# tuplex/tuplex

Measured on AMD Instinct MI355X. Metric: rows/s, higher is better.
Workload: dtype u8; 1 GPU; zillow-Z1 csv->map/withColumn/filter->tocsv (BASELINE.json configs[1]); mb_per_gpu=1024, sink=csv-device-resident

## Files before the change

__graft_entry__.py:

```python
import os
import subprocess
import sys

HERE = os.path.dirname(os.path.abspath(__file__))
sys.path.insert(0, HERE)


def build() -> None:
    from tuplex_amd.csrc import build as nb
    nb.build()
    import tuplex_amd
    subprocess.check_call([sys.executable, os.path.abspath(__file__),
                           "precompile"], cwd=HERE,
                          stdin=subprocess.DEVNULL)
    mk = os.path.join(HERE, "oracle", "Makefile")
    if os.path.exists(mk):
        subprocess.check_call(["make", "-C", os.path.join(HERE, "oracle"), "-s"])


def _precompile() -> None:
    from tests import (chunk_order_pipelines, fused_pipelines, pipelines,
                       regex_pipelines, vocab_pipelines)
    pipelines._COLLECTOR = jobs = []
    try:
        pipelines.precompile_all(verbose=False)
        pipelines.precompile_extra(verbose=False)
        regex_pipelines.precompile(verbose=False)
        chunk_order_pipelines.precompile(verbose=False)
        vocab_pipelines.precompile(verbose=False)
        fused_pipelines.precompile(verbose=False)
    finally:
        pipelines._COLLECTOR = None
    n = pipelines.compile_collected(jobs)
    print("precompiled %d stage kernels into tuplex_amd/.kernel_cache" % n)


def smoke() -> None:
    import tuplex_amd
    from oracle import pyoracle
    from tests.pipelines import PIPELINES, apply_ops

    name, data, columns, ops = PIPELINES[0]
    ctx = tuplex_amd.Context()
    ds = apply_ops(ctx.parallelize(data, columns=columns), ops)
    got = ds.collect()
    assert ds._last_outcome.mode == "gpu", (
        "smoke must run the GPU path, got %r (%s)"
        % (ds._last_outcome.mode, ds._last_outcome.fallback_reason))
    ref = pyoracle.run_pipeline(data, ops, columns=columns)
    assert got == ref["output"], (got, ref["output"])
    assert ds.exception_counts == ref["exception_counts"]
    print("smoke ok:", got)


if __name__ == "__main__":
    if len(sys.argv) > 1 and sys.argv[1] == "smoke":
        smoke()
    elif len(sys.argv) > 1 and sys.argv[1] == "precompile":
        _precompile()
    else:
        build()
```

tuplex_amd/codegen.py:

```python
import os
from typing import List, Optional, Tuple

from . import ttypes as T


class CodegenError(Exception):
    """Stage outside the GPU vocabulary -> caller falls back to interpreter mode
    (the reference's fallback for non-compilable stages)."""


_RT_HEADER_CACHE = None


def runtime_header() -> str:
    global _RT_HEADER_CACHE
    if _RT_HEADER_CACHE is None:
        path = os.path.join(os.path.dirname(os.path.abspath(__file__)),
                            "csrc", "tpx_rt.hip.h")
        _RT_HEADER_CACHE = open(path).read()
    return _RT_HEADER_CACHE


_RE_HEADER_CACHE = None


def regex_header() -> str:
    global _RE_HEADER_CACHE
    if _RE_HEADER_CACHE is None:
        path = os.path.join(os.path.dirname(os.path.abspath(__file__)),
                            "csrc", "tpx_re.hip.h")
        _RE_HEADER_CACHE = open(path).read()
    return _RE_HEADER_CACHE


_FMT_HEADER_CACHE = None


def fmt_header() -> str:
    global _FMT_HEADER_CACHE
    if _FMT_HEADER_CACHE is None:
        path = os.path.join(os.path.dirname(os.path.abspath(__file__)),
                            "csrc", "tpx_fmt.hip.h")
        _FMT_HEADER_CACHE = open(path).read()
    return _FMT_HEADER_CACHE


def _ctype(t):
    base = T.deopt(t)
    if base in (T.I64,):
        return "long long"
    if base == T.F64:
        return "double"
    if base == T.BOOL:
        return "bool"
    if base == T.STR:
        return "tstr"
    raise CodegenError("unsupported column type %r" % (t,))


def _esc(s: str) -> str:
    out = []
    for ch in s:
        o = ord(ch)
        if ch == "\\":
            out.append("\\\\")
        elif ch == '"':
            out.append('\\"')
        elif 32 <= o < 127:
            out.append(ch)
        else:
            for b in ch.encode("utf-8"):
                out.append("\\x%02x" % b)
    return "".join(out)


class _Emitter:
    def __init__(self):
        self.lines: List[str] = []
        self.indent = 1
        self.ctr = 0
        self.scopes = [{}]
        self.key_scopes = [{}]

    def w(self, line):
        self.lines.append("    " * self.indent + line)

    def fresh(self, pfx="t"):
        self.ctr += 1
        return "%s%d" % (pfx, self.ctr)

    def push(self):
        self.scopes.append({})
        self.key_scopes.append({})

    def pop(self):
        self.scopes.pop()
        self.key_scopes.pop()

    def lookup(self, node):
        for s in reversed(self.scopes):
            if id(node) in s:
                return s[id(node)]
        return None

    def memo(self, node, val):
        self.scopes[-1][id(node)] = val
        return val

    def lookup_key(self, key):
        for s in reversed(self.key_scopes):
            if key in s:
                return s[key]
        return None

    def memo_key(self, key, val):
        self.key_scopes[-1][key] = val
        return val


class StageCodegen:

    def __init__(self, sp, source="mem", sink="mem", csv_info=None,
                 fusion_groups=None):
        self.sp = sp
        self.source = source
        self.sink = sink
        self.csv_info = csv_info or {}
        self.lits = {}
        self.lit_defs = []
        self.join_defs = []
        self.fmt_progs = {}
        self.fmt_defs = []
        self.uses_fmt = False
        self.scan_registry = {}
        self.fusion_groups = fusion_groups
        self.fused_done = set()
        import os as _os
        self.split = (source == "csv"
                      and not (csv_info or {}).get("text_mode")
                      and _os.environ.get("TPX_SPLIT", "0") == "1")
        self.park_copy = _os.environ.get("TPX_PARK_COPY", "0") == "1"
        self.fused = False
        self.fused_window = False

    def lit(self, s: str) -> str:
        if s not in self.lits:
            name = "lit%d" % len(self.lits)
            self.lits[s] = name
            b = s.encode("utf-8")
            self.lit_defs.append(
                '__device__ const char %s[%d] = "%s";' % (name, len(b) + 1, _esc(s)))
        return "tstr{%s, %d}" % (self.lits[s], len(s.encode("utf-8")))

    def re_prog(self, prog) -> str:
        if not hasattr(self, "re_progs"):
            self.re_progs = {}
            self.re_defs = []
        key = tuple(prog.words)
        if key not in self.re_progs:
            name = "re_prog%d" % len(self.re_progs)
            self.re_progs[key] = name
            self.re_defs.append("__device__ const int %s[%d] = {%s};"
                                % (name, len(key), ",".join(map(str, key))))
        return self.re_progs[key]

    def fmt_prog(self, items) -> Tuple[str, int, str]:
        from .udf import fmtspec
        self.uses_fmt = True
        key = tuple(items)
        if key not in self.fmt_progs:
            words, blob = fmtspec.encode(items)
            name = "fmt_prog%d" % len(self.fmt_progs)
            self.fmt_defs.append("__device__ const int %s[%d] = {%s};"
                                 % (name, len(words), ",".join(map(str, words))))
            self.fmt_progs[key] = (name, len(items),
                                   self.lit(blob.decode("utf-8")) + ".p")
        return self.fmt_progs[key]

    @staticmethod
    def _struct_key(node):
        out = [node["op"], repr(node.get("v")), node.get("i"), node.get("w"),
               repr(node["t"])]
        for a in node["args"]:
            out.append(StageCodegen._struct_key(a))
        return tuple(out)

    _NONSTRICT = {"if", "and", "or", "const", "input", "mktuple",
                  "strfind", "contains"}

    def emit_expr(self, em: _Emitter, node, row_ctx, opid) -> Tuple[str, Optional[str]]:
        hit = em.lookup(node)
        if hit is not None:
            return hit
        if node["op"] not in self._NONSTRICT:
            pv = self._peephole(em, node, row_ctx, opid)
            if pv is not None:
                return em.memo(node, pv)
# ... 985 lines not shown
        if op == "concat":
            return self._qfree_and(self._qfree_node(a[0], env),
                                   self._qfree_node(a[1], env))
        if op == "center":
            x, _ = ev(a[0])
            w, _ = ev(a[1])
            f = None
            if len(a) == 3:
                f, _ = ev(a[2])
            r = em.fresh("s")
            em.w("tstr %s = tpx_center(heap, %s, (long long)%s, %s, &_ec);"
                 % (r, x, w, f if f else 'tstr{" ", 1}'))
            self._check(em, opid)
            return (r, None)
        if op == "strmul":
            return self._qfree_node(a[0], env)
        if op == "replace":
            rep = a[2]
            rep_ok = (rep["op"] == "const" and isinstance(rep.get("v"), str)
                      and self._qfree_static_str(rep["v"]))
            return self._qfree_and(self._qfree_node(a[0], env),
                                   True if rep_ok else False)
        if op == "to_str":
            from . import ttypes as _T
            if _T.deopt(a[0]["t"]) == _T.STR:
                return self._qfree_node(a[0], env)
            return True
        if op == "fmt_int":
            return True
        if op == "if":
            return self._qfree_and(self._qfree_node(a[1], env),
                                   self._qfree_node(a[2], env))
        return False

    def _thread_qfree(self):
        sp = self.sp
        if getattr(sp, "agg_expr", None) is not None or \
                self._dup_join_op() is not None:
            return None
        env = []
        for i, t in enumerate(sp.input_types):
            if T.deopt(t) == T.STR:
                env.append(frozenset([i]) if self.source == "csv"
                           and not self.csv_info.get("text_mode") else False)
            else:
                env.append(True)
        for op in sp.ops:
            if op.kind == "map":
                if op.tir["op"] == "mktuple":
                    env = [self._qfree_node(el, env) for el in op.tir["args"]]
                else:
                    env = [self._qfree_node(op.tir, env)]
            elif op.kind == "filter":
                pass
            elif op.kind == "withColumn":
                v = self._qfree_node(op.tir, env)
                cols = op.in_columns or ["column%d" % i
                                         for i in range(len(env))]
                if op.col in cols:
                    i = cols.index(op.col)
                    env = env[:i] + [v] + env[i + 1:]
                else:
                    env = env + [v]
            elif op.kind == "mapColumn":
                i = op.in_columns.index(op.col)
                env = env[:i] + [self._qfree_node(op.tir, [env[i]])] + \
                    env[i + 1:]
            elif op.kind == "selectColumns":
                env = [env[i] for i in op.sel_idxs]
            elif op.kind == "renameColumn":
                pass
            elif op.kind == "join":
                rrows, rcols, lki, rki, how = op.join
                right = []
                for j in range(len(rcols)):
                    if j == rki:
                        continue
                    right.append(all(not isinstance(r[j], str)
                                     or self._qfree_static_str(r[j])
                                     for r in rrows))
                env = [env[i] for i in range(len(env)) if i != lki] + \
                    [env[lki]] + right
            else:
                return None
        return env

    def _qfree_cond(self, q):
        if q is True:
            return "true"
        if q is False or q is None:
            return None
        if self.split:
            if any(i >= 64 for i in q):
                return None
            return " && ".join("(((_dirty >> %d) & 1) == 0)" % i
                               for i in sorted(q))
        return " && ".join("((cl%d.flags & 9) == 0)" % i for i in sorted(q))

    def _dup_join_op(self):
        sp = self.sp
        if sp.ops and sp.ops[-1].kind == "join" and \
                getattr(sp.ops[-1], "join_dup", False):
            return sp.ops[-1]
        return None

    def generate(self) -> Tuple[str, str]:
        sp = self.sp
        in_types = sp.input_types
        out_types = sp.gpu_output_types if getattr(sp, "agg_expr", None) is not None \
            else sp.output_types

        dup_op = self._dup_join_op()
        store_types = out_types
        if dup_op is not None:
            n_leftout = len(dup_op.in_types)
            store_types = list(out_types[:n_leftout]) + [T.I64, T.I64]

        body = _Emitter()
        self.row_ctx_initial = []
        for i, t in enumerate(in_types):
            nv = ("c%d_n" % i) if T.is_opt(t) else None
            self.row_ctx_initial.append(("c%d" % i, t, nv))
        final_rc = self.emit_process(body)

        out_fields = []
        for k, t in enumerate(store_types):
            ct = _ctype(t)
            out_fields.append("    %s o%d;" % (ct, k))
            if T.is_opt(t):
                out_fields.append("    bool o%d_n;" % k)
        n_rc = len(store_types) - (2 if dup_op is not None else 0)
        for k, ((v, t, nv), ot) in enumerate(zip(final_rc[:n_rc],
                                                 store_types[:n_rc])):
            cast = "(double)" if T.deopt(ot) == T.F64 and T.deopt(t) in (T.I64, T.BOOL) else ""
            body.w("o.o%d = %s(%s);" % (k, cast, v))
            if T.is_opt(ot):
                body.w("o.o%d_n = %s;" % (k, nv if nv else "false"))
        if dup_op is not None:
            body.w("o.o%d = (long long)%s;" % (n_rc, self.jdup["start_var"]))
            body.w("o.o%d = (long long)%s;" % (n_rc + 1, self.jdup["cnt_var"]))
        body.w("o.keep = true;")
        body.w("return 0;")

        self.store_types = store_types
        self.full_out_types = out_types
        import os as _os
        self.fused = (self.sink == "csv" and self.source != "col"
                      and not self.split and dup_op is None
                      and getattr(sp, "agg_expr", None) is None
                      and _os.environ.get("TPX_FUSED_SINK", "1") != "0"
                      and _os.environ.get("TPX_GEN_BODY") != "1")
        self.fused_window = (self.fused and
                             _os.environ.get("TPX_FUSED_WINDOW", "1") != "0")
        if self.split:
            main_src = ("#define TPX_SPAN_CAP %d\n" % self.SPAN_CAP +
                        self._parse_kernel(in_types) + "\n\n" +
                        self._main_kernel_split(in_types, store_types))
        else:
            main_src = self._main_kernel(in_types, store_types)
        if self.fused:
            write_src = ""
        elif dup_op is None:
            write_src = self._write_kernel(out_types)
        elif self.sink == "mem":
            write_src = self._write_kernel_mem_dup(out_types, store_types)
        else:
            write_src = self._write_kernel_csv_dup(out_types, store_types)
        src = [
            "// generated by tuplex_amd.codegen — stage %s" % sp.signature(),
            runtime_header(),
            "",
        ] + self._re_section() + self._fmt_section() + self.lit_defs + \
            self.join_defs + [
            "",
            "struct Out {",
        ] + out_fields + [
            "    bool keep;",
            "};",
            "",
            self._process_signature(in_types),
            "    int _ec = 0;",
        ] + body.lines + [
            "}",
            "",
            main_src,
            write_src,
        ]
        desc = self._desc(in_types, store_types)
        return "\n".join(src), desc

    def _re_section(self):
        if not getattr(self, "re_defs", None):
            return []
        return [regex_header(), ""] + self.re_defs

    def _fmt_section(self):
        if not self.uses_fmt:
            return []
        return [fmt_header(), ""] + self.fmt_defs

    def _process_signature(self, in_types):
        params = []
        for i, t in enumerate(in_types):
            params.append("%s c%d" % (_ctype(t), i))
            if T.is_opt(t):
                params.append("bool c%d_n" % i)
        params.append("TpxHeap& heap")
        params.append("Out& o")
        return ("__device__ __forceinline__ long long tpx_process(%s) {"
                % ", ".join(params))

    SPAN_CAP = 16344

    def _main_kernel(self, in_types, out_types):
        if self.source == "col":
            return self._main_kernel_col(in_types, out_types)
        L = []
        L.append("#define TPX_SPAN_CAP %d" % self.SPAN_CAP)
        import os as _os
        lb = int(_os.environ.get("TPX_MAIN_LB", "2"))
        bound = " __launch_bounds__(128, %d)" % lb if lb else ""
        L.append('extern "C" __global__ void%s tpx_stage_main(' % bound)
        L.append("    const unsigned char* __restrict__ in_data,")
        L.append("    const long long* __restrict__ in_offs,")
        L.append("    long long n, long long row0,")
        L.append("    char* heap_base, unsigned long long* heap_cursor,"
                 " unsigned long long heap_cap,")
        L.append("    unsigned char* __restrict__ keep, long long* __restrict__ keep01,")
        L.append("    long long* __restrict__ sizes,")
        L.append("    long long* exc_buf, unsigned long long* exc_count,"
                 " unsigned long long exc_cap,")
        L.append("    void** outv) {")
        if self.fused_window:
            L.append("#define TPX_WCAP %d" % self.WRITE_CAP)
            L.append("  __shared__ __attribute__((aligned(16))) char"
                     " smem[2 * TPX_SPAN_CAP + 80 + 2 * TPX_WCAP];"
                     "  // 40 KiB: 4 blocks/CU")
        else:
            L.append("  __shared__ char smem[2 * TPX_SPAN_CAP + 80];  // 2 waves per 128-thread block, 32 KiB")
        L.append("  TpxHeap heap{heap_base, heap_cursor, heap_cap, nullptr, nullptr};")
        L.append("  int lane = threadIdx.x & 63;")
        L.append("  int wid = threadIdx.x >> 6;")
        L.append("  char* wave_lds = smem + wid * TPX_SPAN_CAP;")
        if self.fused_window:
            L.append("  char* wave_out = smem + 2 * TPX_SPAN_CAP + 80"
                     " + wid * TPX_WCAP;")
        L.append("  long long wave_stride = (long long)gridDim.x * (blockDim.x >> 6);")
        L.append("  long long nwaves = (n + 63) >> 6;")
        if self.fused:
            L.append("  const TpxCsvSink _K = *(const TpxCsvSink*)outv;")
        L.append("  for (long long wb = (long long)blockIdx.x * (blockDim.x >> 6) + wid;"
                 " wb < nwaves; wb += wave_stride) {")
        L.append("    long long r0 = wb << 6;")
        L.append("    long long rhi = r0 + 64 < n ? r0 + 64 : n;")
        L.append("    long long span_start = in_offs[r0] & ~15LL;  // align staging window")
        L.append("    long long span_end = in_offs[rhi];")
        L.append("    long long span = span_end - span_start;")
        L.append("    bool staged = span <= TPX_SPAN_CAP;")
        L.append("    if (staged) {")
        L.append("      for (long long k = (long long)lane * 16; k < span; k += 64 * 16) {")
        L.append("        if (k + 16 <= span)")
        L.append("          *(uint4*)(wave_lds + k) = *(const uint4*)((const char*)in_data + span_start + k);")
        L.append("        else")
        L.append("          for (long long j = k; j < span; ++j)")
        L.append("            wave_lds[j] = ((const char*)in_data)[span_start + j];")
        L.append("      }")
        L.append("    }")
        L.append("    long long i = r0 + lane;")
        if self.fused:
            L.append("    bool _live = i < rhi;")
        else:
            L.append("    if (i >= rhi) continue;")
        if _os.environ.get("TPX_GEN_BODY") == "1":
            L.extend(self._row_body(in_types, out_types, lds="gen"))
        else:
            L.append("    if (staged) {")
            L.extend("  " + ln
                     for ln in self._row_body(in_types, out_types, lds=True))
            L.append("    } else {")
            L.extend("  " + ln
                     for ln in self._row_body(in_types, out_types, lds=False))
            L.append("    }")
        L.append("  }")
        L.append("}")
        return "\n".join(L)


    def _parse_kernel(self, in_types):
        used = getattr(self.sp, "used_source_cols", None)
        if used is None:
            used = set(range(len(in_types)))
        L = []
        L.append('extern "C" __global__ void __launch_bounds__(128, 2)'
                 ' tpx_stage_parse(')
        L.append("    const unsigned char* __restrict__ in_data,")
        L.append("    const long long* __restrict__ in_offs,")
        L.append("    long long n, long long row0,")
        L.append("    char* __restrict__ strbuf,"
                 " unsigned long long* __restrict__ str_cursor,")
        L.append("    void** pv, long long* __restrict__ prc_out,")
        L.append("    unsigned long long* __restrict__ dirty_out) {")
        L.append("  __shared__ char smem[2 * TPX_SPAN_CAP + 80];")
        L.append("  int lane = threadIdx.x & 63;")
        L.append("  int wid = threadIdx.x >> 6;")
        L.append("  char* wave_lds = smem + wid * TPX_SPAN_CAP;")
        L.append("  long long wave_stride = (long long)gridDim.x * (blockDim.x >> 6);")
        L.append("  long long nwaves = (n + 63) >> 6;")
        L.append("  for (long long wb = (long long)blockIdx.x * (blockDim.x >> 6) + wid;"
                 " wb < nwaves; wb += wave_stride) {")
        L.append("    long long r0 = wb << 6;")
        L.append("    long long rhi = r0 + 64 < n ? r0 + 64 : n;")
        L.append("    long long span_start = in_offs[r0] & ~15LL;")
        L.append("    long long span_end = in_offs[rhi];")
        L.append("    long long span = span_end - span_start;")
        L.append("    bool staged = span <= TPX_SPAN_CAP;")
        L.append("    if (staged) {")
        L.append("      for (long long k = (long long)lane * 16; k < span; k += 64 * 16) {")
        L.append("        if (k + 16 <= span)")
        L.append("          *(uint4*)(wave_lds + k) = *(const uint4*)((const char*)in_data + span_start + k);")
        L.append("        else")
        L.append("          for (long long j = k; j < span; ++j)")
        L.append("            wave_lds[j] = ((const char*)in_data)[span_start + j];")
        L.append("      }")
        L.append("    }")
        L.append("    long long i = r0 + lane;")
        L.append("    bool _act = i < rhi;")
        L.append("    if (!_act) i = r0;")
        body_store = self._store_parsed(in_types, used)
        L.append("    if (staged) {")
        L.extend("  " + ln for ln in
                 self._load_inputs_csv(in_types, lds=True) + body_store)
        L.append("    } else {")
        L.extend("  " + ln for ln in
                 self._load_inputs_csv(in_types, lds=False) + body_store)
        L.append("    }")
        L.append("  }")
        L.append("}")
        return "\n".join(L)

    def _store_parsed(self, in_types, used):
        str_used = [i for i, t in enumerate(in_types)
                    if i in used and T.deopt(t) == T.STR]
        if not self.park_copy:
            return self._store_parsed_nocopy(in_types, used, str_used)
        L = []
        L.append("    long long _sb = 0;")
        if str_used:
            L.append("    if (_act && !prc) _sb = 8 %s;"
                     % "".join(" + c%d.n" % i for i in str_used))
        L.append("    unsigned long long _v = (unsigned long long)_sb;")
        L.append("    for (int _s = 1; _s < 64; _s <<= 1) {")
        L.append("      unsigned long long _u = __shfl_up(_v, _s);")
        L.append("      if (lane >= _s) _v += _u;")
        L.append("    }")
        L.append("    unsigned long long _off = _v - (unsigned long long)_sb;")
        L.append("    unsigned long long _tot = __shfl(_v, 63);")
        L.append("    unsigned long long _base = 0;")
        L.append("    if (lane == 0 && _tot) _base = atomicAdd(str_cursor, _tot);")
        L.append("    _base = __shfl(_base, 0);")
        L.append("    char* _dst = strbuf + _base + _off;")
        for idx, t in enumerate(in_types):
            if idx not in used:
                continue
            base = T.deopt(t)
            opt = T.is_opt(t)
            if base == T.STR:
                L.append("    if (_act) {")
                L.append("      ((unsigned long long*)pv[%d])[i] ="
                         " (unsigned long long)_dst;" % (3 * idx))
                L.append("      ((int*)pv[%d])[i] = prc ? 0 : (int)c%d.n;"
                         % (3 * idx + 1, idx))
                L.append("      if (!prc) {")
                L.append("        const char* _s = c%d.p; long long _n = c%d.n;"
                         % (idx, idx))
                L.append("        long long _k = 0;")
                L.append("        for (; _k + 8 <= _n; _k += 8)")
                L.append("          *(unsigned long long*)(_dst + _k) ="
                         " *(const unsigned long long*)(_s + _k);")
                L.append("        for (; _k < _n; ++_k) _dst[_k] = _s[_k];")
                L.append("        _dst += _n;")
                L.append("      }")
                L.append("    }")
            elif base == T.F64:
                L.append("    if (_act) ((double*)pv[%d])[i] = c%d;"
                         % (3 * idx, idx))
            else:
                L.append("    if (_act) ((long long*)pv[%d])[i] ="
                         " (long long)c%d;" % (3 * idx, idx))
            if opt:
                L.append("    if (_act) ((unsigned char*)pv[%d])[i] ="
                         " c%d_n ? 1 : 0;" % (3 * idx + 2, idx))
        dirty_bits = ["((unsigned long long)((cl%d.flags & 9) != 0) << %d)"
                      % (i, i) for i in str_used if i < 64]
        L.append("    if (_act) {")
        L.append("      prc_out[i] = prc;")
        L.append("      dirty_out[i] = %s;"
                 % (" | ".join(dirty_bits) if dirty_bits else "0"))
        L.append("    }")
        return L

    def _store_parsed_nocopy(self, in_types, used, str_used):
        L = []
        for idx, t in enumerate(in_types):
            if idx not in used:
                continue
            base = T.deopt(t)
            opt = T.is_opt(t)
            if base == T.STR:
                L.append("    if (_act) {")
                L.append("      tstr _g%d = c%d;" % (idx, idx))
                if True:
                    L.append("      _g%d = tpx_to_global(_g%d, wave_lds,"
                             " wave_lds + TPX_SPAN_CAP, in_data,"
                             " span_start);" % (idx, idx))
                L.append("      ((unsigned long long*)pv[%d])[i] ="
                         " (unsigned long long)_g%d.p;" % (3 * idx, idx))
                L.append("      ((int*)pv[%d])[i] = prc ? 0 : (int)_g%d.n;"
                         % (3 * idx + 1, idx))
                L.append("    }")
            elif base == T.F64:
# ... 184 lines not shown
        L.append("    if (!rc) rc = tpx_process(%s, heap, o);" % ", ".join(args))
        L.append("    if (rc != 0) {")
        L.append("      unsigned long long e = atomicAdd(exc_count, 1ULL);")
        L.append("      if (e < exc_cap) {")
        L.append("        exc_buf[e*5+0] = row0 + i;")
        L.append("        exc_buf[e*5+1] = rc & 0xFFFFFFFFLL;")
        L.append("        exc_buf[e*5+2] = rc >> 32;")
        if self.source == "col":
            L.append("        exc_buf[e*5+3] = 0;")
            L.append("        exc_buf[e*5+4] = 0;")
        else:
            L.append("        exc_buf[e*5+3] = in_offs[i];")
            L.append("        exc_buf[e*5+4] = in_offs[i+1];")
        L.append("      }")
        L.append("      keep[i] = 0; keep01[i] = 0; sizes[i] = 0; continue;")
        L.append("    }")
        L.append("    if (!o.keep) { keep[i] = 0; keep01[i] = 0; sizes[i] = 0; continue; }")
        L.extend(self._store_columnar(out_types, lds))
        if self._dup_join_op() is not None:
            L.append("    keep[i] = 1; keep01[i] = o.o%d;"
                     % (len(out_types) - 1))
        elif self.sink == "mem":
            L.append("    keep[i] = 1; keep01[i] = 1;")
        else:
            L.append("    keep[i] = (unsigned char)(1 | (_anyq ? 0 : 2));"
                     " keep01[i] = 1;")
        return L

    def _load_inputs_col(self, in_types):
        used = getattr(self.sp, "used_source_cols", None)
        L = ["    long long prc = 0;"]
        L.append("    const void* const* ct = (const void* const*)in_data;")
        for idx, t in enumerate(in_types):
            base = T.deopt(t)
            opt = T.is_opt(t)
            if used is not None and idx not in used:
                if opt:
                    L.append("    bool c%d_n = false;  // unused (pushdown)" % idx)
                if base == T.STR:
                    L.append("    tstr c%d{(const char*)in_data, 0};" % idx)
                elif base == T.I64:
                    L.append("    long long c%d = 0;" % idx)
                elif base == T.F64:
                    L.append("    double c%d = 0.0;" % idx)
                else:
                    L.append("    bool c%d = false;" % idx)
                continue
            if opt:
                L.append("    bool c%d_n = ((const unsigned char*)ct[%d])[i]"
                         " != 0;" % (idx, 3 * idx + 2))
            if base == T.STR:
                L.append("    long long c%d_o = ((const long long*)ct[%d])[i];"
                         % (idx, 3 * idx))
                L.append("    tstr c%d{(const char*)ct[%d] + c%d_o,"
                         " ((const long long*)ct[%d])[i + 1] - c%d_o};"
                         % (idx, 3 * idx + 1, idx, 3 * idx, idx))
                guard = ("!prc && !c%d_n" % idx) if opt else "!prc"
                L.append("    if (%s && !tpx_ascii(c%d)) prc = 7;" % (guard, idx))
            elif base == T.I64:
                L.append("    long long c%d = ((const long long*)ct[%d])[i];"
                         % (idx, 3 * idx))
            elif base == T.F64:
                L.append("    double c%d = ((const double*)ct[%d])[i];"
                         % (idx, 3 * idx))
            elif base == T.BOOL:
                L.append("    bool c%d = ((const unsigned char*)ct[%d])[i]"
                         " != 0;" % (idx, 3 * idx))
            else:
                raise CodegenError("columnar input type %r" % (t,))
        return L

    def _load_inputs_mem(self, in_types, lds=True):
        L = ["    long long prc = 0;  // no pre-parse errors on the mem path"]
        if lds == "gen":
            L.append("    unsigned long long _rwa = staged ?"
                     " (unsigned long long)wave_lds + (unsigned long long)(in_offs[i]"
                     " - span_start) : (unsigned long long)(in_data +"
                     " in_offs[i]);")
            L.append('    asm volatile("" : "+v"(_rwa));'
                     "  // opaque: block addrspace re-inference")
            L.append("    const unsigned char* row ="
                     " (const unsigned char*)_rwa;")
        elif lds:
            L.append("    const unsigned char* row ="
                     " (const unsigned char*)(wave_lds + (in_offs[i] - span_start));")
        else:
            L.append("    const unsigned char* row = in_data + in_offs[i];")
        n_opt = sum(1 for t in in_types if T.is_opt(t))
        bitmap_size = ((n_opt + 63) // 64) * 8 if n_opt else 0
        L.append("    // deserialize (bitmap %dB, %d slots)" % (bitmap_size, len(in_types)))
        if bitmap_size:
            for w in range(bitmap_size // 8):
                L.append("    unsigned long long bm%d = ((const unsigned long long*)row)[%d];" % (w, w))
        opt_counter = 0
        for idx, t in enumerate(in_types):
            base = T.deopt(t)
            slot = "((const long long*)(row + %d))[%d]" % (bitmap_size, idx)
            if T.is_opt(t):
                L.append("    bool c%d_n = (bm%d >> %d) & 1;"
                         % (idx, opt_counter // 64, opt_counter % 64))
                opt_counter += 1
            if base == T.I64:
                L.append("    long long c%d = %s;" % (idx, slot))
            elif base == T.BOOL:
                L.append("    bool c%d = %s != 0;" % (idx, slot))
            elif base == T.F64:
                L.append("    double c%d = __longlong_as_double(%s);" % (idx, slot))
            elif base == T.STR:
                L.append("    long long info%d = %s;" % (idx, slot))
                L.append("    tstr c%d{(const char*)(row + %d + %d) + (info%d & 0xFFFFFFFFLL),"
                         " (info%d >> 32) - 1};" % (idx, bitmap_size, idx * 8, idx, idx))
                if T.is_opt(t):
                    L.append("    if (c%d_n) c%d = tstr{(const char*)row, 0};" % (idx, idx))
                L.append("    if (!prc && !tpx_ascii(c%d)) prc = 7;" % idx)
            else:
                raise CodegenError("input type %r" % (t,))
        return L

    def _load_inputs_csv(self, in_types, lds=True):
        if self.csv_info.get("text_mode"):
            return self._load_inputs_text(in_types, lds)
        nc = len(in_types)
        null_values = self.csv_info.get("null_values", [""])
        delim = self.csv_info.get("delimiter", ",")
        assert len(delim) == 1
        delim_c = "'\\t'" if delim == "\t" else "'%s'" % delim
        L = []
        L.append("    long long prc = 0;")
        if lds == "gen":
            L.append("    unsigned long long _rpa = staged ?"
                     " (unsigned long long)wave_lds + (unsigned long long)(in_offs[i]"
                     " - span_start) : (unsigned long long)((const char*)"
                     "in_data + in_offs[i]);")
            L.append("    unsigned long long _rea = staged ?"
                     " (unsigned long long)wave_lds + (unsigned long long)(in_offs[i+1]"
                     " - span_start) : (unsigned long long)((const char*)"
                     "in_data + in_offs[i+1]);")
            L.append('    asm volatile("" : "+v"(_rpa), "+v"(_rea));'
                     "  // opaque: block addrspace re-inference")
            L.append("    const char* rp = (const char*)_rpa;")
            L.append("    const char* rend = (const char*)_rea;")
        elif lds:
            L.append("    const char* rp = wave_lds + (in_offs[i] - span_start);")
            L.append("    const char* rend = wave_lds + (in_offs[i+1] - span_start);")
        else:
            L.append("    const char* rp = (const char*)in_data + in_offs[i];")
            L.append("    const char* rend = (const char*)in_data + in_offs[i+1];")
        L.append("    if (rend > rp && rend[-1] == '\\n') --rend;")
        L.append("    if (rend > rp && rend[-1] == '\\r') --rend;")
        chk_comma = 1 if delim != "," else 0
        L.append("    tpx_mwalk S; tpx_mw_init(S, rp, rend);")
        L.append("    bool avail = true;")
        L.append("    int badf = 0;")

        def null_check(idx):
            cv = "tstr{cl%d.p, cl%d.n}" % (idx, idx)
            checks = " || ".join("tpx_streq(%s, %s)" % (cv, self.lit(nv))
                                 for nv in null_values) or "false"
            return checks

        used = getattr(self.sp, "used_source_cols", None)
        for idx, t in enumerate(in_types):
            base = T.deopt(t)
            opt = T.is_opt(t)
            L.append("    tpx_cell cl%d{rp, 0, 0};" % idx)
            L.append("    if (!prc) {")
            L.append("      if (!avail) prc = %d;  // CSV_UNDERRUN" % 20)
            L.append("      else { tpx_mw_cell(S, &cl%d, %s, %d);"
                     " avail = S.more; badf |= cl%d.flags; }"
                     % (idx, delim_c, chk_comma, idx))
            L.append("    }")
            if used is not None and idx not in used:
                if opt:
                    L.append("    bool c%d_n = false;  // unused (pushdown)" % idx)
                if base == T.STR:
                    L.append("    tstr c%d{cl%d.p, cl%d.n};" % (idx, idx, idx))
                    L.append("    if (prc) c%d = tstr{rp, 0};" % idx)
                elif base == T.I64:
                    L.append("    long long c%d = 0;  // unused (pushdown)" % idx)
                elif base == T.F64:
                    L.append("    double c%d = 0.0;  // unused (pushdown)" % idx)
                else:
                    L.append("    bool c%d = false;  // unused (pushdown)" % idx)
                continue
            if opt:
                L.append("    bool c%d_n = !prc && (%s);" % (idx, null_check(idx)))
            guard = ("!prc && !c%d_n" % idx) if opt else "!prc"
            if base == T.STR:
                L.append("    tstr c%d{cl%d.p, cl%d.n};" % (idx, idx, idx))
                L.append("    if (prc) c%d = tstr{rp, 0};" % idx)
                if opt:
                    L.append("    if (c%d_n) c%d = tstr{rp, 0};" % (idx, idx))
            elif base == T.I64:
                L.append("    long long c%d = 0;" % idx)
                L.append("    if (%s && tpx_cell_i64(cl%d, &c%d) != 0) prc = %d;"
                         % (guard, idx, idx, 70))
            elif base == T.F64:
                L.append("    double c%d = 0.0;" % idx)
                L.append("    if (%s && tpx_cell_f64(cl%d, &c%d) != 0) prc = %d;"
                         % (guard, idx, idx, 70))
            elif base == T.BOOL:
                L.append("    bool c%d = false;" % idx)
                L.append("    if (%s && tpx_cell_bool(cl%d, &c%d) != 0) prc = %d;"
                         % (guard, idx, idx, 70))
            else:
                raise CodegenError("csv input type %r" % (t,))
        L.append("    if (!prc && avail) prc = %d;  // CSV_OVERRUN" % 21)
        L.append("    if (!prc && (badf & 6)) prc = %d;  // BADPARSE (escapes/structure -> host)" % 70)
        L.append("    if (!prc && S.hib) prc = %d;  // NCV" % 7)
        return L

    def _load_inputs_text(self, in_types, lds=True):
        assert len(in_types) == 1
        t = in_types[0]
        null_values = self.csv_info.get("null_values", [])
        L = ["    long long prc = 0;"]
        if lds == "gen":
            L.append("    unsigned long long _rpa = staged ?"
                     " (unsigned long long)wave_lds + (unsigned long long)(in_offs[i]"
                     " - span_start) : (unsigned long long)((const char*)"
                     "in_data + in_offs[i]);")
            L.append("    unsigned long long _rea = staged ?"
                     " (unsigned long long)wave_lds + (unsigned long long)(in_offs[i+1]"
                     " - span_start) : (unsigned long long)((const char*)"
                     "in_data + in_offs[i+1]);")
            L.append('    asm volatile("" : "+v"(_rpa), "+v"(_rea));'
                     "  // opaque: block addrspace re-inference")
            L.append("    const char* rp = (const char*)_rpa;")
            L.append("    const char* rend = (const char*)_rea;")
        elif lds:
            L.append("    const char* rp = wave_lds + (in_offs[i] - span_start);")
            L.append("    const char* rend = wave_lds + (in_offs[i+1] - span_start);")
        else:
            L.append("    const char* rp = (const char*)in_data + in_offs[i];")
            L.append("    const char* rend = (const char*)in_data + in_offs[i+1];")
        L.append("    if (rend > rp && rend[-1] == '\\n') --rend;")
        L.append("    if (rend > rp && rend[-1] == '\\r') --rend;")
        L.append("    tstr c0{rp, rend - rp};")
        L.append("    if (!tpx_ascii(c0)) prc = %d;  // row ASCII gate (NCV)" % 7)
        if T.is_opt(t):
            checks = " || ".join("tpx_streq(c0, %s)" % self.lit(nv)
                                 for nv in null_values) or "false"
            L.append("    bool c0_n = %s;" % checks)
            L.append("    if (c0_n) c0 = tstr{rp, 0};")
        return L

    def _store_columnar(self, out_types, lds=True):
        L = []
        import os as _os2
        _wd2 = int(_os2.environ.get("TPX_WDBG", "0"))
        if _wd2 in (7, 8, 9, 10, 11) and lds == "gen":
            if _wd2 == 7:
                L.append("    { tstr _t = o.o1; if (staged) _t = tpx_to_global"
                         "(_t, wave_lds, wave_lds + TPX_SPAN_CAP, in_data,"
                         " span_start); o.o0 = (long long)_t.p; }  // DBG")
            elif _wd2 == 9:
                L.append("    o.o0 = (long long)o.o1.p;  // DBG pre-translate")
            elif _wd2 == 8:
                L.append("    o.o0 = (long long)wave_lds;  // DBG")
            elif _wd2 == 10:
                L.append("    o.o0 = (long long)in_data;  // DBG")
            elif _wd2 == 11:
                L.append("    o.o0 = staged ? span_start : -1;  // DBG")
        if self.sink != "mem":
            if self._dup_join_op() is not None:
                L.extend(self._csv_size_dup(out_types))
            else:
                L.extend(self._csv_size(out_types))
        for k, t in enumerate(out_types):
            base = T.deopt(t)
            if base == T.STR:
                import os as _os
                _wd = int(_os.environ.get("TPX_WDBG", "0"))
                if _wd == 3:
                    L.append("    o.o%d = tstr{(const char*)in_data, 0};" % k)
                if lds == "gen":
                    L.append("    if (staged) o.o%d = tpx_to_global(o.o%d,"
                             " wave_lds, wave_lds + TPX_SPAN_CAP, in_data,"
                             " span_start);" % (k, k))
                elif lds and lds != "park":
                    L.append("    o.o%d = tpx_to_global(o.o%d, wave_lds,"
                             " wave_lds + TPX_SPAN_CAP, in_data, span_start);"
                             % (k, k))
                L.append("    ((unsigned long long*)outv[%d])[i] = (unsigned long long)o.o%d.p;"
                         % (3 * k, k))
                L.append("    ((int*)outv[%d])[i] = (int)o.o%d.n;" % (3 * k + 1, k))
            elif base == T.F64:
                L.append("    ((double*)outv[%d])[i] = o.o%d;" % (3 * k, k))
            else:
                L.append("    ((long long*)outv[%d])[i] = (long long)o.o%d;" % (3 * k, k))
            if T.is_opt(t):
                L.append("    ((unsigned char*)outv[%d])[i] = o.o%d_n ? 1 : 0;"
                         % (3 * k + 2, k))
        dup_op = self._dup_join_op()
        if self.sink == "mem" and dup_op is not None:
            full = self.full_out_types
            n_opt = sum(1 for t in full if T.is_opt(t))
            bitmap = ((n_opt + 63) // 64) * 8 if n_opt else 0
            has_var = any(T.is_varlen(t) for t in full)
            fixed = bitmap + 8 * len(full) + (8 if has_var else 0)
            n_left = len(dup_op.in_types)
            jd = self.jdup
            nm = jd["nm"]
            L.append("    long long lvar = 0;")
            for k in range(n_left):
                if T.is_varlen(full[k]):
                    if T.is_opt(full[k]):
                        L.append("    if (!o.o%d_n) lvar += o.o%d.n + 1;"
                                 % (k, k))
                    else:
                        L.append("    lvar += o.o%d.n + 1;" % k)
            L.append("    long long rvar = 0;")
            L.append("    for (int _d = 0; _d < o.o%d; ++_d) {"
                     % (len(out_types) - 1))
            L.append("      int _fi = o.o%d < 0 ? 0 : (int)o.o%d + _d;"
                     % (len(out_types) - 2, len(out_types) - 2))
            L.append("      bool _miss = o.o%d < 0;" % (len(out_types) - 2))
            for (j, kindc, has_null) in jd["out_info"]:
                if kindc == "str":
                    cond = "!_miss"
                    if has_null:
                        cond += " && !%s_c%d_null[_fi]" % (nm, j)
                    L.append("      if (%s) rvar += %s_c%d_len[_fi] + 1;"
                             % (cond, nm, j))
            L.append("    }")
            L.append("    sizes[i] = (long long)o.o%d * (%d + lvar) + rvar;"
                     % (len(out_types) - 1, fixed))
        elif self.sink == "mem":
            n_opt = sum(1 for t in out_types if T.is_opt(t))
            bitmap = ((n_opt + 63) // 64) * 8 if n_opt else 0
            has_var = any(T.is_varlen(t) for t in out_types)
            fixed = bitmap + 8 * len(out_types) + (8 if has_var else 0)
            L.append("    long long sz = %d;" % fixed)
            for k, t in enumerate(out_types):
                if T.is_varlen(t):
                    if T.is_opt(t):
                        L.append("    if (!o.o%d_n) sz += o.o%d.n + 1;" % (k, k))
                    else:
                        L.append("    sz += o.o%d.n + 1;" % k)
            L.append("    sizes[i] = sz;")
        return L

    def _csv_size(self, out_types):
        decl = ("", "") if self.fused else ("long long ", "bool ")
        L = ["    %ssz = %d;  // delimiters + newline" % (decl[0], len(out_types))]
        L.append("    %s_anyq = false;" % decl[1])
        qfree = self._thread_qfree()
        for k, t in enumerate(out_types):
            base = T.deopt(t)
            if base == T.STR:
                qc = self._qfree_cond(qfree[k]) if qfree is not None else None
                pre = ""
                if T.is_opt(t):
                    L.append("    if (!o.o%d_n) {" % k)
                    pre = "  "
                if qc == "true":
                    L.append(pre + "    sz += o.o%d.n;" % k)
                elif qc is not None:
                    L.append(pre + "    if (%s) { sz += o.o%d.n; }" % (qc, k))
# ... 580 lines not shown
```

Before: 865.5 million rows/s.

## Build a wave-parallel CSV cell index during LDS staging

```diff
diff --git a/__graft_entry__.py b/__graft_entry__.py
--- a/__graft_entry__.py
+++ b/__graft_entry__.py
@@ -19,8 +19,9 @@
 
 
 def _precompile() -> None:
-    from tests import (chunk_order_pipelines, fused_pipelines, pipelines,
-                       regex_pipelines, vocab_pipelines)
+    from tests import (cellindex_pipelines, chunk_order_pipelines,
+                       fused_pipelines, pipelines, regex_pipelines,
+                       vocab_pipelines)
     pipelines._COLLECTOR = jobs = []
     try:
         pipelines.precompile_all(verbose=False)
@@ -29,6 +30,7 @@
         chunk_order_pipelines.precompile(verbose=False)
         vocab_pipelines.precompile(verbose=False)
         fused_pipelines.precompile(verbose=False)
+        cellindex_pipelines.precompile(verbose=False)
     finally:
         pipelines._COLLECTOR = None
     n = pipelines.compile_collected(jobs)
diff --git a/tuplex_amd/codegen.py b/tuplex_amd/codegen.py
--- a/tuplex_amd/codegen.py
+++ b/tuplex_amd/codegen.py
@@ -43,6 +43,18 @@
                             "csrc", "tpx_fmt.hip.h")
         _FMT_HEADER_CACHE = open(path).read()
     return _FMT_HEADER_CACHE
+
+
+_CI_HEADER_CACHE = None
+
+
+def ci_header() -> str:
+    global _CI_HEADER_CACHE
+    if _CI_HEADER_CACHE is None:
+        path = os.path.join(os.path.dirname(os.path.abspath(__file__)),
+                            "csrc", "tpx_ci.hip.h")
+        _CI_HEADER_CACHE = open(path).read()
+    return _CI_HEADER_CACHE
 
 
 def _ctype(t):
@@ -1334,6 +1346,14 @@
                       and _os.environ.get("TPX_GEN_BODY") != "1")
         self.fused_window = (self.fused and
                              _os.environ.get("TPX_FUSED_WINDOW", "1") != "0")
+        self.cell_index = (
+            self.source == "csv" and not self.split
+            and not self.csv_info.get("text_mode")
+            and self.csv_info.get("delimiter", ",") == ","
+            and 1 <= len(in_types) <= self.CI_MAX_COLS
+            and _os.environ.get("TPX_GEN_BODY") != "1"
+            and _os.environ.get("TPX_CELL_INDEX",
+                                self.CELL_INDEX_DEFAULT) != "0")
         if self.split:
             main_src = ("#define TPX_SPAN_CAP %d\n" % self.SPAN_CAP +
                         self._parse_kernel(in_types) + "\n\n" +
@@ -1352,7 +1372,8 @@
             "// generated by tuplex_amd.codegen — stage %s" % sp.signature(),
             runtime_header(),
             "",
-        ] + self._re_section() + self._fmt_section() + self.lit_defs + \
+        ] + self._ci_section() + self._re_section() + self._fmt_section() + \
+            self.lit_defs + \
             self.join_defs + [
             "",
             "struct Out {",
@@ -1376,6 +1397,14 @@
             return []
         return [regex_header(), ""] + self.re_defs
 
+    def _ci_section(self):
+        if not self.cell_index:
+            return []
+        return [ci_header(),
+                "static_assert(64 * %d + 1 <= TPX_CI_CAP,"
+                " \"a full batch of well-formed rows fits the index\");"
+                % len(self.sp.input_types), ""]
+
     def _fmt_section(self):
         if not self.uses_fmt:
             return []
@@ -1393,6 +1422,10 @@
                 % ", ".join(params))
 
     SPAN_CAP = 16344
+    CI_BYTES = 4096
+    CI_CAP = (CI_BYTES - 264) // 4
+    CI_MAX_COLS = (CI_CAP - 1) // 64
+    CELL_INDEX_DEFAULT = "1"
 
     def _main_kernel(self, in_types, out_types):
         if self.source == "col":
@@ -1418,6 +1451,10 @@
             L.append("  __shared__ __attribute__((aligned(16))) char"
                      " smem[2 * TPX_SPAN_CAP + 80 + 2 * TPX_WCAP];"
                      "  // 40 KiB: 4 blocks/CU")
+        elif self.cell_index:
+            L.append("  __shared__ __attribute__((aligned(16))) char"
+                     " smem[2 * TPX_SPAN_CAP + 80 + 2 * TPX_CI_BYTES];"
+                     "  // 40 KiB: 4 blocks/CU")
         else:
             L.append("  __shared__ char smem[2 * TPX_SPAN_CAP + 80];  // 2 waves per 128-thread block, 32 KiB")
         L.append("  TpxHeap heap{heap_base, heap_cursor, heap_cap, nullptr, nullptr};")
@@ -1427,6 +1464,14 @@
         if self.fused_window:
             L.append("  char* wave_out = smem + 2 * TPX_SPAN_CAP + 80"
                      " + wid * TPX_WCAP;")
+        if self.cell_index:
+            if self.fused_window:
+                assert self.WRITE_CAP == self.CI_BYTES
+                L.append("  char* wave_ci = wave_out;  // idle until the"
+                         " wave commit")
+            else:
+                L.append("  char* wave_ci = smem + 2 * TPX_SPAN_CAP + 80"
+                         " + wid * TPX_CI_BYTES;")
         L.append("  long long wave_stride = (long long)gridDim.x * (blockDim.x >> 6);")
         L.append("  long long nwaves = (n + 63) >> 6;")
         if self.fused:
@@ -1439,15 +1484,22 @@
         L.append("    long long span_end = in_offs[rhi];")
         L.append("    long long span = span_end - span_start;")
         L.append("    bool staged = span <= TPX_SPAN_CAP;")
-        L.append("    if (staged) {")
-        L.append("      for (long long k = (long long)lane * 16; k < span; k += 64 * 16) {")
-        L.append("        if (k + 16 <= span)")
-        L.append("          *(uint4*)(wave_lds + k) = *(const uint4*)((const char*)in_data + span_start + k);")
-        L.append("        else")
-        L.append("          for (long long j = k; j < span; ++j)")
-        L.append("            wave_lds[j] = ((const char*)in_data)[span_start + j];")
-        L.append("      }")
-        L.append("    }")
+        if self.cell_index:
+            L.append("    bool _ci_ok = false;")
+            L.append("    if (staged)")
+            L.append("      _ci_ok = tpx_ci_stage(wave_lds, wave_ci,"
+                     " (const char*)in_data + span_start, (int)span,"
+                     " (int)(in_offs[r0] - span_start), ',', lane);")
+        else:
+            L.append("    if (staged) {")
+            L.append("      for (long long k = (long long)lane * 16; k < span; k += 64 * 16) {")
+            L.append("        if (k + 16 <= span)")
+            L.append("          *(uint4*)(wave_lds + k) = *(const uint4*)((const char*)in_data + span_start + k);")
+            L.append("        else")
+            L.append("          for (long long j = k; j < span; ++j)")
+            L.append("            wave_lds[j] = ((const char*)in_data)[span_start + j];")
+            L.append("      }")
+            L.append("    }")
         L.append("    long long i = r0 + lane;")
         if self.fused:
             L.append("    bool _live = i < rhi;")
@@ -1938,6 +1990,13 @@
         L.append("    tpx_mwalk S; tpx_mw_init(S, rp, rend);")
         L.append("    bool avail = true;")
         L.append("    int badf = 0;")
+        ci = self.cell_index and lds is True
+        if ci:
+            L.append("    int _rs = (int)(in_offs[i] - span_start);")
+            L.append("    int _e0 = 0;")
+            L.append("    bool _fast = _ci_ok && tpx_ci_row(wave_lds, wave_ci,"
+                     " lane, _rs, (int)(in_offs[i+1] - span_start),"
+                     " (int)(rend - wave_lds), (int)span, %d, &_e0);" % nc)
 
         def null_check(idx):
             cv = "tstr{cl%d.p, cl%d.n}" % (idx, idx)
@@ -1951,7 +2010,14 @@
             opt = T.is_opt(t)
             L.append("    tpx_cell cl%d{rp, 0, 0};" % idx)
             L.append("    if (!prc) {")
-            L.append("      if (!avail) prc = %d;  // CSV_UNDERRUN" % 20)
+            if ci:
+                L.append("      if (_fast) tpx_ci_cell(wave_lds, wave_ci, _e0,"
+                         " %d, %d, _rs, (int)(rend - wave_lds), &cl%d);"
+                         % (idx, nc, idx))
+                L.append("      else if (!avail) prc = %d;  // CSV_UNDERRUN"
+                         % 20)
+            else:
+                L.append("      if (!avail) prc = %d;  // CSV_UNDERRUN" % 20)
             L.append("      else { tpx_mw_cell(S, &cl%d, %s, %d);"
                      " avail = S.more; badf |= cl%d.flags; }"
                      % (idx, delim_c, chk_comma, idx))
@@ -1991,6 +2057,8 @@
                          % (guard, idx, idx, 70))
             else:
                 raise CodegenError("csv input type %r" % (t,))
+        if ci:
+            L.append("    if (_fast) avail = false;")
         L.append("    if (!prc && avail) prc = %d;  // CSV_OVERRUN" % 21)
         L.append("    if (!prc && (badf & 6)) prc = %d;  // BADPARSE (escapes/structure -> host)" % 70)
         L.append("    if (!prc && S.hib) prc = %d;  // NCV" % 7)
diff --git a/tuplex_amd/csrc/tpx_ci.hip.h b/tuplex_amd/csrc/tpx_ci.hip.h
--- /dev/null
+++ b/tuplex_amd/csrc/tpx_ci.hip.h
@@ -0,0 +1,226 @@
+
+#define TPX_CI_BYTES 4096
+#define TPX_CI_RF_OFF 0
+#define TPX_CI_BAD_OFF 136
+#define TPX_CI_ENT_OFF 264
+#define TPX_CI_CAP ((TPX_CI_BYTES - TPX_CI_ENT_OFF) / 4)
+#define TPX_CI_NONE 0xFFFFu
+
+__device__ __forceinline__ unsigned tpx_ci_zero32(unsigned x) {
+    return ~(x | ((x | 0x80808080u) - 0x01010101u)) & 0x80808080u;
+}
+
+__device__ __forceinline__ unsigned tpx_ci_pack4(unsigned h) {
+    unsigned x = h >> 7;
+    x |= x >> 7;
+    x |= x >> 14;
+    return x & 0xFu;
+}
+
+struct tpx_ci_cls { unsigned q, s, n, r, h; };
+
+__device__ __forceinline__ void tpx_ci_classify(unsigned w0, unsigned w1,
+                                                unsigned w2, unsigned w3,
+                                                char delim, unsigned valid,
+                                                tpx_ci_cls* c) {
+    const unsigned one = 0x01010101u;
+    unsigned pq = one * (unsigned)'"', pd = one * (unsigned char)delim;
+    unsigned pn = one * (unsigned)'\n', pr = one * (unsigned)'\r';
+    unsigned w[4] = {w0, w1, w2, w3};
+    unsigned q = 0, s = 0, n = 0, r = 0, h = 0;
+    #pragma unroll
+    for (int d = 0; d < 4; ++d) {
+        unsigned v = w[d];
+        unsigned zn = tpx_ci_zero32(v ^ pn);
+        q |= tpx_ci_pack4(tpx_ci_zero32(v ^ pq)) << (4 * d);
+        s |= tpx_ci_pack4(tpx_ci_zero32(v ^ pd) | zn) << (4 * d);
+        n |= tpx_ci_pack4(zn) << (4 * d);
+        r |= tpx_ci_pack4(tpx_ci_zero32(v ^ pr)) << (4 * d);
+        h |= tpx_ci_pack4(v & 0x80808080u) << (4 * d);
+    }
+    c->q = q & valid; c->s = s & valid; c->n = n & valid;
+    c->r = r & valid; c->h = h & valid;
+}
+
+__device__ __forceinline__ unsigned tpx_ci_inq(unsigned q16, unsigned par) {
+    unsigned x = q16;
+    x ^= x << 1; x ^= x << 2; x ^= x << 4; x ^= x << 8;
+    x <<= 1;
+    if (par) x = ~x;
+    return x & 0xFFFFu;
+}
+
+__device__ __forceinline__ void tpx_ci_scatter(char* ci, int k, unsigned s16,
+                                               unsigned n16, unsigned q16,
+                                               unsigned ord, unsigned nl,
+                                               unsigned qc0) {
+    unsigned* ent = (unsigned*)(ci + TPX_CI_ENT_OFF);
+    unsigned short* rf = (unsigned short*)(ci + TPX_CI_RF_OFF);
+    while (s16) {
+        int j = __ffs((int)s16) - 1;
+        unsigned isnl = (n16 >> j) & 1u;
+        unsigned qc = qc0 + (unsigned)__popc(q16 & ((1u << j) - 1u));
+        if (ord < TPX_CI_CAP)
+            ent[ord] = (unsigned)(k + j) | (isnl << 15) | (qc << 16);
+        ++ord;
+        if (isnl) {
+            ++nl;
+            if (nl <= 64 && ord <= TPX_CI_CAP) rf[nl] = (unsigned short)ord;
+        }
+        s16 &= s16 - 1;
+    }
+}
+
+__device__ __forceinline__ int tpx_ci_row(const char* base, const char* ci,
+                                          int r, int rs, int re, int rend,
+                                          int span, int ncols, int* e0_out) {
+    const unsigned* ent = (const unsigned*)(ci + TPX_CI_ENT_OFF);
+    const unsigned short* rf = (const unsigned short*)(ci + TPX_CI_RF_OFF);
+    const unsigned long long* bad =
+        (const unsigned long long*)(ci + TPX_CI_BAD_OFF);
+    if (re <= rs) return 0;
+    unsigned e0 = rf[r], e1 = rf[r + 1];
+    if (e0 == TPX_CI_NONE || e1 == TPX_CI_NONE) return 0;
+    if (e1 != e0 + (unsigned)ncols) return 0;
+    unsigned q = 0;
+    if (e0 == 0) {
+        if (r != 0) return 0;
+    } else {
+        unsigned pe = ent[e0 - 1];
+        if (!(pe & 0x8000u) || (int)(pe & 0x3FFFu) != rs - 1) return 0;
+        q = pe >> 16;
+    }
+    unsigned le = ent[e1 - 1];
+    int lp = (int)(le & 0x3FFFu);
+    if (le & 0x8000u) {
+        if (lp != re - 1) return 0;
+    } else {
+        if (lp != re || re != span) return 0;
+    }
+    int b0 = rs >> 4, b1 = (re - 1) >> 4;
+    for (int w = b0 >> 6; w <= (b1 >> 6); ++w) {
+        int lo = w == (b0 >> 6) ? (b0 & 63) : 0;
+        int hi = w == (b1 >> 6) ? (b1 & 63) : 63;
+        unsigned long long m = (~0ULL << lo) & (~0ULL >> (63 - hi));
+        if (bad[w] & m) return 0;
+    }
+    int cs = rs;
+    for (int k = 0; k < ncols; ++k) {
+        unsigned e = ent[e0 + (unsigned)k];
+        int ce = k == ncols - 1 ? rend : (int)(e & 0x3FFFu);
+        unsigned nq = ((e >> 16) - q) & 0xFFFFu;
+        if (nq && (nq != 2 || ce - cs < 2 || base[cs] != '"' ||
+                   base[ce - 1] != '"'))
+            return 0;
+        q = e >> 16;
+        cs = (int)(e & 0x3FFFu) + 1;
+    }
+    *e0_out = (int)e0;
+    return 1;
+}
+
+__device__ __forceinline__ void tpx_ci_cell(const char* base, const char* ci,
+                                            int e0, int k, int ncols, int rs,
+                                            int rend, tpx_cell* c) {
+    const unsigned* ent = (const unsigned*)(ci + TPX_CI_ENT_OFF);
+    unsigned e = ent[e0 + k];
+    int cs = rs;
+    unsigned q = 0;
+    if (e0 + k > 0) {
+        unsigned pe = ent[e0 + k - 1];
+        cs = (int)(pe & 0x3FFFu) + 1;
+        q = pe >> 16;
+    }
+    int ce = k == ncols - 1 ? rend : (int)(e & 0x3FFFu);
+    if (((e >> 16) - q) & 0xFFFFu) {
+        c->p = base + cs + 1; c->n = ce - cs - 2; c->flags = 1 | 8;
+    } else {
+        c->p = base + cs; c->n = ce - cs; c->flags = 0;
+    }
+}
+
+#ifndef TPX_HOST_TEST
+__device__ __forceinline__ unsigned tpx_wave_exscan32(unsigned v, int lane) {
+    unsigned x = v;
+    for (int o = 1; o < 64; o <<= 1) {
+        unsigned y = __shfl_up(x, o);
+        if (lane >= o) x += y;
+    }
+    return x - v;
+}
+
+__device__ __forceinline__ bool tpx_ci_stage(char* wave_lds, char* ci,
+                                             const char* src, int span, int lo,
+                                             char delim, int lane) {
+    unsigned* ent = (unsigned*)(ci + TPX_CI_ENT_OFF);
+    unsigned short* rf = (unsigned short*)(ci + TPX_CI_RF_OFF);
+    unsigned long long* bad = (unsigned long long*)(ci + TPX_CI_BAD_OFF);
+    rf[lane + 1] = (unsigned short)TPX_CI_NONE;
+    if (lane == 0) rf[0] = 0;
+    unsigned car_ord = 0, car_nl = 0, car_q = 0;
+    bool pend = false;
+    unsigned long long below = (1ull << lane) - 1ull;
+    int trip = 0;
+    uint4 pre = make_uint4(0, 0, 0, 0);
+    if (lane * 16 + 16 <= span) pre = *(const uint4*)(src + lane * 16);
+    for (int kb = 0; kb < span; kb += 64 * 16, ++trip) {
+        int k = kb + lane * 16;
+        unsigned w0 = 0, w1 = 0, w2 = 0, w3 = 0;
+        if (k + 16 <= span) {
+            uint4 v = pre;
+            if (k + 64 * 16 + 16 <= span)
+                pre = *(const uint4*)(src + k + 64 * 16);
+            *(uint4*)(wave_lds + k) = v;
+            w0 = v.x; w1 = v.y; w2 = v.z; w3 = v.w;
+        } else {
+            unsigned long long a = 0, b = 0;
+            for (int j = k; j < span; ++j) {
+                unsigned char ch = (unsigned char)src[j];
+                wave_lds[j] = (char)ch;
+                int t = j - k;
+                if (t < 8) a |= (unsigned long long)ch << (8 * t);
+                else b |= (unsigned long long)ch << (8 * (t - 8));
+            }
+            w0 = (unsigned)a; w1 = (unsigned)(a >> 32);
+            w2 = (unsigned)b; w3 = (unsigned)(b >> 32);
+        }
+        int nv = span - k; nv = nv < 0 ? 0 : (nv > 16 ? 16 : nv);
+        int nl_ = lo - k; nl_ = nl_ < 0 ? 0 : (nl_ > 16 ? 16 : nl_);
+        unsigned valid = ((1u << nv) - 1u) & ~((1u << nl_) - 1u);
+        tpx_ci_cls c;
+        tpx_ci_classify(w0, w1, w2, w3, delim, valid, &c);
+        unsigned pq = (unsigned)__popc(c.q);
+        unsigned long long oddm = __ballot(pq & 1u);
+        unsigned par = (car_q ^ (unsigned)__popcll(oddm & below)) & 1u;
+        unsigned inq = tpx_ci_inq(c.q, par);
+        unsigned s16 = c.s & ~inq, n16 = c.n & ~inq;
+        unsigned ps = (unsigned)__popc(s16), pn = (unsigned)__popc(n16);
+        unsigned ex = tpx_wave_exscan32(ps | (pn << 11) | (pq << 22), lane);
+        unsigned xs = ex & 0x7FFu, xn = (ex >> 11) & 0x7FFu, xq = ex >> 22;
+        unsigned long long nlf = __ballot(n16 & 1u);
+        unsigned nxt = lane < 63 ? (unsigned)((nlf >> (lane + 1)) & 1ull) : 0u;
+        unsigned badr = c.r & ~((n16 >> 1) | (nxt << 15));
+        bool mypend = lane == 63 && (badr & 0x8000u);
+        if (lane == 63) badr &= 0x7FFFu;
+        unsigned long long bw = __ballot(c.h != 0 || badr != 0);
+        if (lane == 0) {
+            if (pend && !(nlf & 1ull)) bad[trip - 1] |= 1ull << 63;
+            bad[trip] = bw;
+        }
+        pend = __ballot(mypend) != 0;
+        tpx_ci_scatter(ci, k, s16, n16, c.q, car_ord + xs, car_nl + xn,
+                       car_q + xq);
+        car_ord += (unsigned)__builtin_amdgcn_readlane((int)(xs + ps), 63);
+        car_nl += (unsigned)__builtin_amdgcn_readlane((int)(xn + pn), 63);
+        car_q += (unsigned)__builtin_amdgcn_readlane((int)(xq + pq), 63);
+    }
+    if (pend && lane == 0) bad[trip - 1] |= 1ull << 63;
+    bool ok = car_ord < TPX_CI_CAP;
+    if (ok && car_nl < 64 && lane == 0) {
+        ent[car_ord] = (unsigned)span | (car_q << 16);
+        rf[car_nl + 1] = (unsigned short)(car_ord + 1);
+    }
+    __builtin_amdgcn_wave_barrier();
+    return ok;
+}
+#endif
```

New measurement: 913.2 million rows/s (median of 6 runs). 5.5% higher.
